# Mordentary/RayTracer-Cuda

Measured on AMD Instinct MI355X. Metric: Mrays/sec + frame wall-clock, Cornell+bunny 2560×1440 2000spp 20bounce, higher is better.
Workload: dtype f32

## Files before the change

### include/crt_hip.h

```cpp
#ifndef CRT_HIP_H
#define CRT_HIP_H

#include <stddef.h>
#include <stdint.h>

#ifdef __cplusplus
extern "C" {
#endif

#define CRT_ABI_VERSION 3

enum crt_status {
    CRT_OK = 0,
    CRT_ERR_INVALID_ARGUMENT = -1,
    CRT_ERR_HIP = -2,
    CRT_ERR_OUT_OF_MEMORY = -3,
    CRT_ERR_NO_DEVICE = -4,
    CRT_ERR_UNSUPPORTED = -5
};

enum crt_material_type { CRT_LAMBERTIAN = 0, CRT_METAL = 1, CRT_DIELECTRIC = 2, CRT_DIFFUSE_LIGHT = 3 };

typedef struct crt_material_desc {
    int32_t type;
// ... 250 lines not shown
int  crt_renderer_render(crt_renderer* r, const crt_scene* scene, int spp, int max_bounces, unsigned flags, void* stream);
int  crt_renderer_resolve(crt_renderer* r, float scale, void* stream);
int  crt_renderer_render_frame(crt_renderer* r, const crt_scene* scene, void* stream);
int  crt_renderer_synchronize(crt_renderer* r, void* stream);
int  crt_renderer_read_linear(crt_renderer* r, float* host_out);
int  crt_renderer_read_rgba8(crt_renderer* r, uint8_t* host_out);
int  crt_renderer_read_rng(crt_renderer* r, uint32_t* host_out);
int  crt_renderer_write_linear(crt_renderer* r, const float* host_in);
int  crt_renderer_get_counters(crt_renderer* r, crt_work_counters* out);
int  crt_renderer_get_schedule_stats(crt_renderer* r, unsigned long long* out3);
int  crt_renderer_get_section_profile(crt_renderer* r, unsigned long long* out7);
int  crt_renderer_get_section_profile_ex(crt_renderer* r, unsigned long long* out, int n);
float* crt_renderer_linear_device_ptr(crt_renderer* r);
int crt_renderer_attach_linear(crt_renderer* r, float* device_ptr);
uint8_t* crt_renderer_rgba_device_ptr(crt_renderer* r);
uint32_t* crt_renderer_rng_device_ptr(crt_renderer* r);
float crt_renderer_last_kernel_ms(crt_renderer* r);
int crt_renderer_last_schedule(crt_renderer* r, float out[4]);
int crt_renderer_last_timings(crt_renderer* r, float out[3]);
#define CRT_TIMING_RING 32
int crt_renderer_timing_history(crt_renderer* r, int back, float out[3]);
const char* crt_renderer_last_kernel_name(const crt_renderer* r);
int crt_renderer_last_launch_frozen(const crt_renderer* r);

int crt_build_mesh_bvh(int device, const float* positions, uint32_t vertex_count, uint32_t* indices,
                       int32_t* face_materials, uint32_t index_count, crt_bvh_node_desc* nodes, int32_t* node_count,
                       float mesh_box[6], float* build_ms);

int crt_selftest_math(const float* a, const float* b, int n, float* out, double* out_f64);
int crt_selftest_rcp(uint32_t lo_bits, uint32_t hi_bits, unsigned long long* mismatches, uint32_t* first_bad);
int crt_selftest_sqrt(uint32_t lo_bits, uint32_t hi_bits, unsigned long long* mismatches, uint32_t* first_bad);
int crt_selftest_unit(const float* in, int n, float* out);
int crt_selftest_uv_div(int dim, unsigned long long* mismatches);
int crt_selftest_scan(const int* in, int n_waves, int* out);
int crt_selftest_geometry(int kind, const float* in, int n, const crt_camera_desc* cam, int width, int height,
                          uint32_t* rng, float* out);
int crt_selftest_rng(unsigned long long seed, const unsigned long long* subseq, int n, int n_draw,
                     uint32_t* state_out , float* uniforms_out );
int crt_selftest_tile_schedule(crt_renderer* r, const uint32_t* pix_cost, int stride, int key_mode, int shard, int shards,
                               int xcd_regions, unsigned long long* stats_out);
int crt_selftest_pixel_order(crt_renderer* r, int kind, const uint32_t* in, int shard, int shards);
int crt_selftest_schedule_buffer(crt_renderer* r, int which, uint32_t* out, int64_t capacity, int64_t* n);

#ifdef __cplusplus
}
#endif
// ... 2 lines not shown
```

### raytracer-cuda_amd/crt_amd/__init__.py

```python
from __future__ import annotations

import ctypes as C
from dataclasses import dataclass

import numpy as np

from . import _lib
from ._lib import CameraDesc, CrtError, SceneDesc, SceneStats, WorkCounters, build, check, check_host

RENDER_ACCUMULATE = 1
RENDER_COUNT_WORK = 2

BENCH_CAMERA = dict(aspect=16.0 / 9.0, vfov=80.0, pos=(0.0, 0.0, 0.3), up=(0.0, 1.0, 0.0),
                    aperture=0.000001, focus=0.3, yaw=-90.0, pitch=0.0)


def _p(a: np.ndarray):
    return a.ctypes.data_as(C.c_void_p)


def camera(spp: int = 1, aspect=16.0 / 9.0, vfov=80.0, pos=(0.0, 0.0, 0.3), up=(0.0, 1.0, 0.0),
           aperture=0.000001, focus=0.3, yaw=-90.0, pitch=0.0) -> CameraDesc:
    d = CameraDesc()
    check_host(_lib.host().crth_camera(C.c_float(aspect), C.c_float(vfov), _p(np.asarray(pos, np.float32)),
# ... 334 lines not shown
    def _borrow(cls, handle, width: int, height: int, device: int, owner):
        r = cls.__new__(cls)
        r.h, r.width, r.height, r.device, r._owned, r._owner = C.c_void_p(handle), width, height, device, False, owner
        return r

    def close(self):
        if getattr(self, "h", None) and _lib is not None:
            if getattr(self, "_owned", True):
                _lib.hip().crt_renderer_destroy(self.h)
            self.h = None

    __del__ = close

    def init_rand(self, seed: int = 41, subsequence_base: int = 0, stream=None):
        check(_lib.hip().crt_renderer_init_rand(self.h, int(seed), int(subsequence_base), stream), "init_rand")

    def set_schedule(self, probe_spp: int = -1, min_spp: int = 64, tile_key: int = 2, probe_stride: int = 0):
        flags = ((int(tile_key) & 0xf) << 16) | ((int(probe_stride) & 0xf) << 20)
        check(_lib.hip().crt_renderer_set_schedule(self.h, int(probe_spp), int(min_spp), flags), "set_schedule")

    def set_critical_tiles(self, tiles: int = -1, lanes: int = 16):
        check(_lib.hip().crt_renderer_set_critical_tiles(self.h, int(tiles), int(lanes)), "set_critical_tiles")

    def set_top_levels(self, levels: int = -1):
        check(_lib.hip().crt_renderer_set_top_levels(self.h, int(levels)), "set_top_levels")

    def set_pixel_shard(self, shard: int = 0, shards: int = 1):
        check(_lib.hip().crt_renderer_set_pixel_shard(self.h, int(shard), int(shards)), "set_pixel_shard")

    def set_kernel_variant(self, variant: int):
        check(_lib.hip().crt_renderer_set_kernel_variant(self.h, int(variant)), "set_kernel_variant")

    def set_occupancy_target(self, waves_per_simd: int):
        check(_lib.hip().crt_renderer_set_occupancy_target(self.h, int(waves_per_simd)), "set_occupancy_target")

    def set_regen_threshold(self, lanes: int):
        check(_lib.hip().crt_renderer_set_regen_threshold(self.h, int(lanes)), "set_regen_threshold")

    def set_stack_lds(self, entries: int):
        check(_lib.hip().crt_renderer_set_stack_lds(self.h, int(entries)), "set_stack_lds")

    def set_camera(self, cam: CameraDesc):
        self._cam = cam
        check(_lib.hip().crt_renderer_set_camera(self.h, C.byref(cam)), "set_camera")

    def render(self, scene: Scene, spp: int, max_bounces: int = 20, accumulate=False, count_work=False, stream=None):
# ... 558 lines not shown
```

### raytracer-cuda_amd/crt_amd/_lib.py

```python
from __future__ import annotations

import ctypes as C
import os
import subprocess
from pathlib import Path

PKG_ROOT = Path(__file__).resolve().parents[1]
REPO = PKG_ROOT.parent
LIB_DIR = PKG_ROOT / "lib"
HIP_LIB = Path(os.environ["CRT_HIP_LIB"]) if os.environ.get("CRT_HIP_LIB") else LIB_DIR / "libcrt_hip.so"
HOST_LIB = Path(os.environ["CRT_HOST_LIB"]) if os.environ.get("CRT_HOST_LIB") else LIB_DIR / "libcrt_host.so"


class CrtError(RuntimeError):
    pass


def build(jobs: int = 8) -> None:
    subprocess.run(["make", "-C", str(PKG_ROOT), f"-j{jobs}", "all"], check=True)


class CameraDesc(C.Structure):
    _fields_ = [("origin", C.c_float * 3), ("lower_left", C.c_float * 3), ("horizontal", C.c_float * 3),
                ("vertical", C.c_float * 3), ("right", C.c_float * 3), ("up", C.c_float * 3),
# ... 135 lines not shown
    "crt_renderer_last_kernel_name", "crt_renderer_last_timings", "crt_renderer_last_schedule", "crt_renderer_timing_history",
    "crt_renderer_set_leaf_carry", "crt_renderer_set_xcd_regions", "crt_renderer_set_temporal_order",
    "crt_renderer_set_drain_threshold", "crt_renderer_set_wave_drain",
    "crt_renderer_attach_linear", "crt_renderer_set_kernel_variant", "crt_renderer_get_schedule_stats",
    "crt_renderer_set_regen_threshold", "crt_renderer_set_occupancy_target",
    "crt_build_mesh_bvh", "crt_renderer_set_schedule", "crt_renderer_set_critical_tiles", "crt_renderer_set_pixel_shard",
    "crt_renderer_set_top_levels",
    "crt_selftest_math", "crt_selftest_rng", "crt_selftest_geometry", "crt_selftest_scan", "crt_selftest_rcp",
    "crt_selftest_uv_div", "crt_selftest_sqrt", "crt_selftest_unit",
    "crt_trace_validate_rays", "crt_scene_export_identity", "crt_scene_trace", "crt_scene_occluded",
    "crt_scene_trace_device", "crt_scene_trace_last_stats",
    "crt_renderer_camera_rays_device", "crt_scene_path_step_device", "crt_scene_export_shade_rows",
    "crt_scene_path_advance_device", "crt_path_advance_entries", "crt_renderer_render_wavefront",
    "crt_scene_trace_indirect_device", "crt_scene_path_advance_indirect_device", "crt_renderer_render_wavefront_queued",
    "crt_scene_path_finish_device", "crt_renderer_render_wavefront_finish",
    "crt_selftest_tile_schedule", "crt_selftest_pixel_order", "crt_selftest_schedule_buffer",
    "crt_renderer_render_adaptive", "crt_renderer_resolve_adaptive", "crt_renderer_read_tile_spp",
    "crt_renderer_read_tile_error", "crt_renderer_read_adaptive_prev", "crt_selftest_adaptive_plan",
    "crt_renderer_compute_guides", "crt_renderer_denoise", "crt_renderer_resolve_denoised",
    "crt_renderer_read_denoised", "crt_renderer_read_guides", "crt_renderer_denoised_device_ptr", "crt_selftest_denoise",
    "crt_renderer_denoise_iteration_ms", "crt_debug_live_allocations", "crt_renderer_last_launch_frozen",
    "crt_renderer_reproject", "crt_renderer_reset_history", "crt_renderer_denoise_history", "crt_renderer_resolve_history",
    "crt_renderer_read_history", "crt_renderer_history_device_ptr", "crt_selftest_reproject",
]
OPTIONAL_SYMBOLS = ("crt_renderer_camera_rays_device", "crt_scene_path_step_device", "crt_scene_export_shade_rows",
                    "crt_scene_path_advance_device", "crt_path_advance_entries", "crt_renderer_render_wavefront",
                    "crt_scene_trace_indirect_device", "crt_scene_path_advance_indirect_device",
                    "crt_renderer_render_wavefront_queued",
                    "crt_scene_path_finish_device", "crt_renderer_render_wavefront_finish",
                    "crt_selftest_tile_schedule", "crt_selftest_pixel_order", "crt_selftest_schedule_buffer",
                    "crt_renderer_render_adaptive", "crt_renderer_resolve_adaptive", "crt_renderer_read_tile_spp",
                    "crt_renderer_read_tile_error", "crt_renderer_read_adaptive_prev", "crt_selftest_adaptive_plan",
                    "crt_renderer_compute_guides", "crt_renderer_denoise", "crt_renderer_resolve_denoised",
                    "crt_renderer_read_denoised", "crt_renderer_read_guides", "crt_renderer_denoised_device_ptr",
                    "crt_selftest_denoise", "crt_renderer_denoise_iteration_ms", "crt_debug_live_allocations",
                    "crt_renderer_last_launch_frozen",
                    "crt_renderer_reproject", "crt_renderer_reset_history", "crt_renderer_denoise_history",
                    "crt_renderer_resolve_history", "crt_renderer_read_history", "crt_renderer_history_device_ptr",
                    "crt_selftest_reproject")

HOST_SYMBOLS = [
    "crth_scene_load", "crth_scene_load_ex", "crth_scene_build_ms", "crth_scene_destroy", "crth_scene_desc", "crth_scene_upload", "crth_scene_upload_ex", "crth_scene_counts",
    "crth_scene_loader_arrays", "crth_camera", "crth_last_error", "crth_encode_image", "crth_write_image",
    "crth_build_mesh_bvh", "crth_camera_create", "crth_camera_update", "crth_camera_get", "crth_camera_destroy",
    "crth_viewer_create", "crth_viewer_frame", "crth_viewer_camera", "crth_viewer_renderer", "crth_viewer_destroy",
    "crth_viewer_set_reproject",
]

_hip = None
_host = None


def _bind_single_runtime() -> None:
    if os.environ.get("CRT_NO_TORCH") == "1":
        return
    try:
        import torch
    except Exception:
        pass


def hip():
# ... 64 lines not shown
            "crt_renderer_render_wavefront": ([P, P, i32, i32, C.c_uint, P, P, P], i32),
            "crt_scene_trace_indirect_device": ([P, P, P, C.c_int64, P, P, P, C.c_uint, P], i32),
            "crt_scene_path_advance_indirect_device": ([P, P, P, P, P, P, C.c_int64, i32, P, P, P, P, P, P, P, P], i32),
            "crt_renderer_render_wavefront_queued": ([P, P, i32, i32, C.c_uint, P, i32, P, P], i32),
            "crt_scene_path_finish_device": ([P, P, P, P, P, C.c_int64, i32, P, P, P, P, P], i32),
            "crt_renderer_render_wavefront_finish": ([P, P, i32, i32, C.c_uint, P, i32, C.c_int64, P, P], i32),
            "crt_selftest_tile_schedule": ([P, P, i32, i32, i32, i32, i32, P], i32),
            "crt_selftest_pixel_order": ([P, i32, P, i32, i32], i32),
            "crt_selftest_schedule_buffer": ([P, i32, P, C.c_int64, P], i32),
            "crt_renderer_render_adaptive": ([P, P, P, i32, C.c_uint, P, P], i32),
            "crt_renderer_resolve_adaptive": ([P, P], i32),
            "crt_renderer_read_tile_spp": ([P, P], i32), "crt_renderer_read_tile_error": ([P, P], i32),
            "crt_renderer_read_adaptive_prev": ([P, P], i32),
            "crt_selftest_adaptive_plan": ([P, P, P, P, i32, i32, f32, P, P], i32),
            "crt_renderer_compute_guides": ([P, P, P, P], i32),
            "crt_renderer_denoise": ([P, P, f32, P, P], i32),
            "crt_renderer_resolve_denoised": ([P, P], i32),
            "crt_renderer_read_denoised": ([P, P], i32), "crt_renderer_read_guides": ([P, P], i32),
            "crt_renderer_denoised_device_ptr": ([P], P),
            "crt_selftest_denoise": ([P, P, P, P, P], i32),
            "crt_renderer_denoise_iteration_ms": ([P, P], i32),
            "crt_debug_live_allocations": ([P, P], i32),
            "crt_renderer_last_launch_frozen": ([P], i32),
            "crt_renderer_reproject": ([P, P, f32, P, P], i32),
            "crt_renderer_reset_history": ([P], i32),
            "crt_renderer_denoise_history": ([P, P, P, P], i32),
            "crt_renderer_resolve_history": ([P, P], i32),
            "crt_renderer_read_history": ([P, P], i32),
            "crt_renderer_history_device_ptr": ([P], P),
            "crt_selftest_reproject": ([P, P, P, P, P, P, P, P], i32),
        }
        for name, (args, res) in sig.items():
            if os.environ.get("CRT_SKIP_ABI_CHECK") and not hasattr(L, name):
                continue
            if name in OPTIONAL_SYMBOLS and not hasattr(L, name):
                continue
            fn = getattr(L, name)
            fn.argtypes = args
            fn.restype = res
        if L.crt_abi_version() != ABI_VERSION and not os.environ.get("CRT_SKIP_ABI_CHECK"):
            raise CrtError(f"{HIP_LIB}: C ABI version {L.crt_abi_version()}, these bindings expect {ABI_VERSION} "
                           "(rebuild the library, or set CRT_SKIP_ABI_CHECK=1 for an A/B run of an older build)")
        _hip = L
    return _hip


# ... 56 lines not shown
```

### raytracer-cuda_amd/csrc/crt_hip.hip

```cpp
#include <hip/hip_runtime.h>

#include <algorithm>
#include <atomic>
#include <chrono>
#include <cstdio>
#include <cstdlib>
#include <cstring>
#include <memory>
#include <mutex>
#include <new>
#include <string>
#include <thread>
#include <type_traits>
#include <vector>

#include "crt_hip.h"
#include "crt_device.h"
#include "crt_devmem.h"
#include "crt_sah.h"
#include "crt/ParallelFor.h"

using namespace crt;

static thread_local std::string g_last_error;
// ... 28 lines not shown
    float sph2[2][12];
    unsigned* err;
    int width, height, spp, max_bounces;
    float rcp_w, rcp_h;
    int fast_uv;
    int accumulate;
    int regen_threshold;
    uint32_t* __restrict__ rng;
    float* __restrict__ sum;
    unsigned long long* __restrict__ counters;
    crt_camera_desc cam;
    const uint32_t* __restrict__ order;
    uint32_t* __restrict__ queue;
    int n_slots;
    int tiles_x;
    uint32_t* __restrict__ probe_cost;
    int probe_stride;
    uint32_t* __restrict__ pix_rays;
    int crit_tiles, crit_threshold;
    int drain_threshold;
    int wave_drain;
    int top_levels;
};

#ifdef CRT_PROFILE_LIVE
__device__ unsigned long long g_live_hist[16];
#endif
#ifdef CRT_PROFILE_PAIRS
__device__ unsigned long long g_pair_hist[32];
#endif

struct TraceCounts {
    uint32_t boxes, tris, spheres, step_slots, round_slots, trace_calls;
    uint64_t cyc_regen, cyc_step, cyc_round, passes;
    uint64_t cyc_shade, cyc_next;
    uint64_t cyc_sph;
    uint64_t cyc_setup, cyc_top, cyc_head;
#ifdef CRT_PROFILE_ROWS
    uint64_t cyc_rows, cyc_prims;
#endif
};
__device__ __forceinline__ uint64_t shader_clock() { return __builtin_amdgcn_s_memtime(); }
__device__ __forceinline__ uint64_t bcast64(uint64_t v, int lane) {
    return ((uint64_t)(uint32_t)__builtin_amdgcn_readlane((int)(v >> 32), lane) << 32) |
           (uint32_t)__builtin_amdgcn_readlane((int)(uint32_t)v, lane);
}
// ... 444 lines not shown
        const unsigned long long kk = L.key[lane];
        const float t = __uint_as_float((unsigned)(kk >> 32));
        const int rank = (int)(0xffffffffu - (unsigned)kk);
        if (kk != ~0ull && better(t, rank, closest, hit)) {
            closest = t;
            hit = rank;
        }
    }
}

#ifndef CRT_CHAIN_RHO
#define CRT_CHAIN_RHO 1.6
#endif
constexpr int STACK_LDS = 16;
#ifndef CRT_STACK6
#define CRT_STACK6 12
#endif
#ifndef CRT_STACK7
#define CRT_STACK7 8
#endif
constexpr int wide_stack_entries(int minw) { return minw >= 7 ? CRT_STACK7 : minw >= 6 ? CRT_STACK6 : STACK_LDS; }
constexpr int REGEN_THRESHOLD_WIDE = 44;
constexpr int WAVE_DRAIN = 48;

struct Wide4 {
    float tmin[4];
    bool hit[4];
};

constexpr float BOX_INV_CLAMP = 0x1p64f;
__device__ __forceinline__ V3 box_inv(V3 inv) {
    return v3(__builtin_amdgcn_fmed3f(inv.x, -BOX_INV_CLAMP, BOX_INV_CLAMP),
              __builtin_amdgcn_fmed3f(inv.y, -BOX_INV_CLAMP, BOX_INV_CLAMP),
              __builtin_amdgcn_fmed3f(inv.z, -BOX_INV_CLAMP, BOX_INV_CLAMP));
}
__device__ __forceinline__ V3 recip3_exact(V3 d) {
    const float ax = fabsf(d.x), ay = fabsf(d.y), az = fabsf(d.z);
    const bool ok = ax >= RCP_FAST_MIN && ax < RCP_FAST_MAX && ay >= RCP_FAST_MIN && ay < RCP_FAST_MAX &&
                    az >= RCP_FAST_MIN && az < RCP_FAST_MAX;
    if (__builtin_amdgcn_ballot_w64(!ok) == 0) return v3(rcp_newton(d.x), rcp_newton(d.y), rcp_newton(d.z));
    __asm__ volatile("");
    return v3(recip_exact_any(d.x), recip_exact_any(d.y), recip_exact_any(d.z));
}
__device__ __forceinline__ V3 sphere_inv(V3 d, V3 binv) {
    if (fabsf(binv.x) == BOX_INV_CLAMP || fabsf(binv.y) == BOX_INV_CLAMP || fabsf(binv.z) == BOX_INV_CLAMP)
        return v3(recip_exact_any(d.x), recip_exact_any(d.y), recip_exact_any(d.z));
// ... 725 lines not shown
    if (hit != h0 && hit >= 0) {
        if (P.n_ray_spheres == 2) {
            const int k = hit == __float_as_int(sph_lds[26]) ? 3 : 0;
            e0 = shd_lds[k];
            e1 = shd_lds[k + 1];
            inv_r = shd_lds[k + 2].x;
            staged = true;
        } else {
            const float4* Rh = P.shade + 3u * (uint32_t)hit;
            e0 = Rh[0];
            e1 = Rh[1];
        }
    }
    shade_rec(S, P, hit, closest, e0, e1, staged, inv_r);
}

#ifdef CRT_PROFILE_WAVE_TIMES
__device__ unsigned long long g_wave_prof[2 * 4 * 65536];
#endif
#ifdef CRT_PROFILE_CRIT_TRACE
__device__ unsigned long long g_crit_trace[2 * 16384];
__device__ unsigned g_wave_hw[2 * 4 * 65536];
#endif

template <int VARIANT> struct KernelShape { static constexpr int waves = VARIANT == 8 || VARIANT == 10 ? 1 : 4; };

template <bool COUNT, int VARIANT, int MINW>
__global__ __launch_bounds__(64 * KernelShape<VARIANT>::waves, MINW) void crt_render_kernel(RenderParams P) {
    constexpr bool FROZEN = VARIANT == 8 && !COUNT;
#include "crt_render_body.inc"
}
template <int VARIANT, int MINW>
__global__ __launch_bounds__(64 * KernelShape<VARIANT>::waves, MINW) void crt_render_open_kernel(RenderParams P) {
    static_assert(VARIANT == 8, "only the plain variant-8 kernels have twins");
    constexpr bool COUNT = false, FROZEN = false;
#include "crt_render_body.inc"
}

struct CompareParams {
    RenderParams A;
    const float4* __restrict__ nodes_b;
    const float4* __restrict__ prims_b;
    int n_nodes_b, n_layouts_b;
    int width_a, width_b;
    int sphere_first_b, n_spheres_b;
    const float4* chain_b;
// ... 1033 lines not shown
    PinnedBuf<unsigned long long> h_probe_stats;
    float last_schedule[4] = {0.f, 0.f, 0.f, 0.f};
    DevBuf<uint32_t> d_rng_cache;
    unsigned long long rng_cache_seed = 0, rng_cache_base = 0;
    bool rng_cache_valid = false;
    int probe_spp = -1;
    int probe_min_spp = 64;
    int tile_key_mode = 2;
    int n_cus = 0;
    int variant = -1;
    unsigned long long diag[3] = {0, 0, 0};
    unsigned long long prof[8] = {0, 0, 0, 0, 0, 0, 0, 0};
    int regen_threshold = 24;
    int regen_threshold_wide = REGEN_THRESHOLD_WIDE;
    int crit_tiles = -1;
    int tile_shard = 0, tile_shards = 1;
    int crit_threshold = 16;
    int top_levels = -1;
    int xcd_regions = 0;
    int probe_stride = 0;
    int temporal = 0;
    int drain_threshold = 0;
    int wave_drain = WAVE_DRAIN;
    DevBuf<uint32_t> d_pix_rays;
    DevBuf<uint32_t> d_tile_order;
    bool pix_rays_valid = false;
    int min_waves = 0;
    DevBuf<uint32_t> d_ovf;
    int stack_lds = STACK_LDS;
    float rcp_w = 1.f, rcp_h = 1.f;
    int fast_uv = 0;
    std::unique_ptr<WavefrontScratch> wavefront;
    std::unique_ptr<AdaptiveState> adaptive;
    std::unique_ptr<DenoiseState> denoise;
    std::unique_ptr<ReprojectState> reproject;
};

namespace {
int use_device(int dev) {
    int n = 0;
    HIP_TRY(hipGetDeviceCount(&n));
    if (n <= 0) return set_error(CRT_ERR_NO_DEVICE, "no HIP device visible");
    if (dev < 0 || dev >= n) return set_error(CRT_ERR_INVALID_ARGUMENT, "device ordinal out of range");
    HIP_TRY(hipSetDevice(dev));
    return CRT_OK;
}
// ... 542 lines not shown
static_assert(render_row_digits(8, true) == 55555677, "variant 8, counting");
static_assert(render_row_digits(10, false) == 55555677 && render_row_digits(10, true) == 55555677, "variant 10");
static_assert(render_row_digits(3, false) == 11145666 && render_row_digits(3, true) == 11145666, "variant 3");
static_assert(render_row_digits(2, false) == 11115668 && render_row_digits(2, true) == 11115668, "variant 2");
static_assert(render_row_digits(0, false) == 11111111 && render_row_digits(0, true) == 11111111, "variant 0");
static_assert(render_row_digits(1, false) == 11111111 && render_row_digits(1, true) == 11111111, "variant 1");

static bool render_launch_frozen(const RenderRow& row, bool cnt, const RenderParams& P, const crt_scene* S) {
    if (!row.open || cnt) return false;
    const int sd = wide_stack_entries(row.w);
    const bool own_bound = S->stack_cap == S->stack_bound;
    const bool stack = own_bound && (P.stack_lds == sd || (S->stack_cap < sd && P.stack_lds == S->stack_cap));
    return stack && P.top_levels == CRT_TOP_LEVELS && P.tree_spheres == 0 && P.n_ray_spheres == 2 && P.n_layouts == 1 &&
           !P.probe_cost && !P.pix_rays && P.wave_drain == WAVE_DRAIN && P.regen_threshold == REGEN_THRESHOLD_WIDE;
}

static int launch_render(crt_renderer* R, const RenderRow& row, bool cnt, dim3 grid, dim3 block, hipStream_t st,
                         const RenderParams& P, const crt_scene* S = nullptr) {
    std::snprintf(R->kernel_name, sizeof R->kernel_name, "crt_render_kernel<%s, %d, %d>", cnt ? "true" : "false",
                  row.variant, row.w);
    if (row.open && !S) return set_error(CRT_ERR_INVALID_ARGUMENT, "launch_render: a variant-8 launch needs its scene");
    R->last_frozen = render_launch_frozen(row, cnt, P, S) ? 1 : 0;
    HIP_TRY(hipEventRecord(R->ev_main, st));
    if (R->last_frozen) {
        RenderParams Q = P;
        Q.stack_lds = wide_stack_entries(row.w);
        hipLaunchKernelGGL(row.plain, grid, block, 0, st, Q);
    } else {
        hipLaunchKernelGGL(cnt ? row.counting : row.open ? row.open : row.plain, grid, block, 0, st, P);
    }
    return CRT_OK;
}

static int ensure_order_buffers(crt_renderer* R, hipStream_t st, size_t n_pix, int n_tiles, bool want_tile_key) {
    if (R->d_order && (R->d_tile_key || !want_tile_key)) return CRT_OK;
    HIP_TRY(hipStreamSynchronize(st));
    if (!R->d_order) {
        HIP_TRY(R->d_order.alloc(std::max(n_pix, (size_t)n_tiles * 64)));
        HIP_TRY(R->d_queue.alloc(1));
        HIP_TRY(R->d_tile_cost.alloc(n_pix));
        HIP_TRY(R->d_order_hist.alloc(ORDER_KEYS));
        HIP_TRY(hipDeviceGetAttribute(&R->n_cus, hipDeviceAttributeMultiprocessorCount, R->device));
    }
    if (want_tile_key && !R->d_tile_key) HIP_TRY(R->d_tile_key.alloc((size_t)n_tiles));
    return CRT_OK;
}

static int sort_descending(crt_renderer* R, hipStream_t st, const uint32_t* keys, int n, uint32_t* out) {
    const unsigned ob = (unsigned)((n + ORDER_ITEMS - 1) / ORDER_ITEMS);
    HIP_TRY(hipMemsetAsync(R->d_order_hist.get(), 0, ORDER_KEYS * 4, st));
    hipLaunchKernelGGL(crt_order_hist_kernel, dim3(ob), dim3(256), 0, st, keys, n, R->d_order_hist.get());
    hipLaunchKernelGGL(crt_order_scan_kernel, dim3(1), dim3(ORDER_KEYS), 0, st, R->d_order_hist.get());
    hipLaunchKernelGGL(crt_order_scatter_kernel, dim3(ob), dim3(256), 0, st, keys, n, R->d_order_hist.get(), out, 0u);
    return CRT_OK;
}

static int order_tiles_by_probe(crt_renderer* R, hipStream_t st, int stride, bool stats, int shard, int shards) {
    const size_t n_pix = (size_t)R->width * R->height;
    const int tiles_x = (R->width + 7) / 8, n_tiles = tiles_x * ((R->height + 7) / 8);
    const dim3 tgrid((n_tiles + 255) / 256), tblock(256);
    if (stats) {
        if (!R->d_probe_stats) {
            HIP_TRY(R->d_probe_stats.alloc(2));
            HIP_TRY(R->h_probe_stats.alloc(2));
// ... 113 lines not shown
        if (variant == 8) {
            P.crit_tiles = R->crit_tiles < 0 ? 4 * R->n_cus : R->crit_tiles;
            P.crit_threshold = R->crit_threshold;
        }
        if (auto_small) {
            HIP_TRY(hipStreamSynchronize(st));
            const double mx = (double)R->h_probe_stats.get()[0];
            const double mine = (double)R->h_probe_stats.get()[1] / shards;
            const double rho = mine > 0 ? mx * (4.0 * R->n_cus * 6) / mine : 0.0;
            if (rho > CRT_CHAIN_RHO) {
                occ = 4;
                P.stack_lds = stack_lds_for(R, S, occ);
            }
            R->last_schedule[0] = (float)rho;
            R->last_schedule[2] = (float)mx;
            R->last_schedule[3] = (float)(mine / std::max(1, n_tiles / shards));
        }
    } else if (shards > 1) {
        shard_tiles_in_row_order(R, st, n_tiles, shard, shards);
        P.order = R->d_order.get();
    }
    if (P.crit_tiles > 0) P.crit_tiles = (P.crit_tiles + shards - 1) / shards;
    if (variant == 8) R->last_schedule[1] = (float)occ;
    const dim3 tgrid((unsigned)((n_tiles - shard + shards - 1) / shards));
    return launch_render(R, RENDER_ROWS[render_row(variant, cnt, occ)], cnt, tgrid, dim3(64), st, P, S);
}

static int order_tile_slots(crt_renderer* R, hipStream_t st) {
    const size_t n_pix = (size_t)R->width * R->height;
    const int tiles_x = (R->width + 7) / 8, n_tiles = tiles_x * ((R->height + 7) / 8);
    const size_t n_tile_slots = (size_t)n_tiles * 64;
    if (R->temporal && !R->d_pix_rays) {
        HIP_TRY(hipStreamSynchronize(st));
        HIP_TRY(R->d_pix_rays.alloc(n_pix));
        HIP_TRY(R->d_tile_order.alloc((size_t)n_tiles));
        if (!R->d_tile_key) HIP_TRY(R->d_tile_key.alloc((size_t)n_tiles));
        R->pix_rays_valid = false;
    }
    const dim3 sgrid((unsigned)((n_tile_slots + 255) / 256));
    if (R->temporal && R->pix_rays_valid) {
        hipLaunchKernelGGL(crt_tile_cost_kernel, dim3((n_tiles + 255) / 256), dim3(256), 0, st, R->d_pix_rays.get(),
                           R->width, R->height, tiles_x, n_tiles, R->d_tile_order.get(), 0, 1, nullptr);
        hipLaunchKernelGGL(crt_tile_neighbour_kernel, dim3((n_tiles + 255) / 256), dim3(256), 0, st,
                           R->d_tile_order.get(), tiles_x, n_tiles, R->d_tile_key.get());
        if (int rc = sort_descending(R, st, R->d_tile_key.get(), n_tiles, R->d_tile_order.get())) return rc;
        hipLaunchKernelGGL(crt_expand_tile_order_kernel, sgrid, dim3(256), 0, st, R->d_tile_order.get(), R->d_order.get(),
// ... 208 lines not shown
int crt_renderer_get_section_profile(crt_renderer* R, unsigned long long* out7) {
    if (!R || !out7) return set_error(CRT_ERR_INVALID_ARGUMENT, "null argument");
    for (int i = 0; i < 7; ++i) out7[i] = R->prof[i];
    return CRT_OK;
}
int crt_renderer_get_section_profile_ex(crt_renderer* R, unsigned long long* out, int n) {
    if (!R || !out || n < 0) return set_error(CRT_ERR_INVALID_ARGUMENT, "bad argument");
    for (int i = 0; i < n && i < 8; ++i) out[i] = R->prof[i];
    return CRT_OK;
}
int crt_renderer_get_schedule_stats(crt_renderer* R, unsigned long long* out3) {
    if (!R || !out3) return set_error(CRT_ERR_INVALID_ARGUMENT, "null argument");
    out3[0] = R->diag[0]; out3[1] = R->diag[1]; out3[2] = R->diag[2];
    return CRT_OK;
}

float* crt_renderer_linear_device_ptr(crt_renderer* R) { return R ? R->d_sum : nullptr; }
uint8_t* crt_renderer_rgba_device_ptr(crt_renderer* R) { return R ? R->d_rgba.get() : nullptr; }
uint32_t* crt_renderer_rng_device_ptr(crt_renderer* R) { return R ? R->d_rng.get() : nullptr; }

const char* crt_renderer_last_kernel_name(const crt_renderer* R) { return R ? R->kernel_name : ""; }
int crt_renderer_last_launch_frozen(const crt_renderer* R) { return R ? R->last_frozen : 0; }

#ifdef CRT_PROFILE_PAIRS
extern "C" int crt_profile_pair_hist(unsigned long long* out32, int reset) {
    if (!out32) return set_error(CRT_ERR_INVALID_ARGUMENT, "bad argument");
    HIP_TRY(hipDeviceSynchronize());
    HIP_TRY(hipMemcpyFromSymbol(out32, HIP_SYMBOL(g_pair_hist), 32 * 8, 0, hipMemcpyDeviceToHost));
    if (reset) {
        static const unsigned long long zero[32] = {};
        HIP_TRY(hipMemcpyToSymbol(HIP_SYMBOL(g_pair_hist), zero, sizeof zero, 0, hipMemcpyHostToDevice));
    }
    return CRT_OK;
}
#endif
#ifdef CRT_PROFILE_LIVE
extern "C" int crt_profile_live_hist(unsigned long long* out16, int reset) {
    if (!out16) return set_error(CRT_ERR_INVALID_ARGUMENT, "bad argument");
    HIP_TRY(hipDeviceSynchronize());
    HIP_TRY(hipMemcpyFromSymbol(out16, HIP_SYMBOL(g_live_hist), 16 * 8, 0, hipMemcpyDeviceToHost));
    if (reset) {
        static const unsigned long long zero[16] = {};
        HIP_TRY(hipMemcpyToSymbol(HIP_SYMBOL(g_live_hist), zero, sizeof zero, 0, hipMemcpyHostToDevice));
    }
    return CRT_OK;
}
// ... 344 lines not shown
```

### raytracer-cuda_amd/csrc/crt_render_body.inc

```
    static_assert(!FROZEN || (VARIANT == 8 && !COUNT), "only the plain variant-8 kernels have a frozen twin");
    if constexpr (FROZEN) {
        constexpr int FROZEN_STACK = wide_stack_entries(MINW);
        __builtin_assume(P.stack_lds == FROZEN_STACK);
        __builtin_assume(P.top_levels == CRT_TOP_LEVELS);
        __builtin_assume(P.tree_spheres == 0);
        __builtin_assume(P.n_ray_spheres == 2);
        __builtin_assume(P.n_layouts == 1);
        __builtin_assume(P.probe_cost == nullptr);
        __builtin_assume(P.pix_rays == nullptr);
        __builtin_assume(P.wave_drain == WAVE_DRAIN);
        __builtin_assume(P.regen_threshold == REGEN_THRESHOLD_WIDE);
    }
#ifdef CRT_PROFILE_WAVE_TIMES
    const unsigned long long prof_t0 = __builtin_amdgcn_s_memrealtime();
#endif
#ifdef CRT_PROFILE_PASS
    const uint64_t prof_life0 = shader_clock();
#endif
    constexpr int WGW = KernelShape<VARIANT>::waves;
    constexpr bool PERSIST = VARIANT == 7;
    constexpr bool TILED = VARIANT == 8;
    constexpr bool TILES = TILED || VARIANT == 10;
    constexpr bool WIDE = VARIANT == 4 || PERSIST || TILED;
    using Lds = std::conditional_t<WIDE, WaveLdsWide, WaveLds>;
// ... 10 lines not shown
            const int k = threadIdx.x & 15;
            const int src = k < 4 ? k : k < 9 ? k + 1 : k == 9 ? 10 : k == 10 ? 4 : -1;
            sph_lds[threadIdx.x] = src < 0 ? 0.f : P.sph2[threadIdx.x >> 4][src];
        }
        if (threadIdx.x >= 32 && threadIdx.x < 38 && P.n_ray_spheres == 2) {
            const uint32_t q = threadIdx.x - 32, sp = q / 3;
            shd_lds[q] = P.shade[3u * (uint32_t)__float_as_int(P.sph2[sp][4]) + q % 3];
        }
        if (TOPN > 0 && threadIdx.x < 8u * TOPN) {
            const uint32_t m = threadIdx.x >> 3, k = threadIdx.x & 7;
            int n = 0;
            if (m > 0) {
                const float4 rm = node_row(P.nodes, node_base(0), 6);
                n = (int)(m - 1) < (__float_as_int(rm.y) & 0xff) ? __float_as_int(rm.x) + (int)(m - 1) : -1;
            }
            if (n >= 0 && n < P.n_nodes) top_lds[threadIdx.x] = node_row(P.nodes, node_base(n), k);
        }
        __syncthreads();
    }
    const int lane = threadIdx.x & 63;
    const int wave = __builtin_amdgcn_readfirstlane(threadIdx.x >> 6);
    int x, y;
    if (TILES) {
        const uint32_t t = P.order ? P.order[blockIdx.x] : blockIdx.x;
        x = (int)(t % (uint32_t)P.tiles_x) * 8 + (lane & 7);
        y = (int)(t / (uint32_t)P.tiles_x) * 8 + (lane >> 3);
    } else {
        x = blockIdx.x * 16 + (wave & 1) * 8 + (lane & 7);
        y = blockIdx.y * 16 + (wave >> 1) * 8 + (lane >> 3);
        if (VARIANT == 4 && P.probe_cost) {
            x *= P.probe_stride;
            y *= P.probe_stride;
        }
    }
    const bool valid = x < P.width && y < P.height;
    const int pix = valid ? y * P.width + x : 0;

    PathState S;
    S.s = Rng{0, 0, 0, 0, 0, 0};
    S.pixel = v3(0.f, 0.f, 0.f);
    S.o = v3(0, 0, 0); S.d = v3(0, 0, 1); S.thr = v3(1, 1, 1);
    S.remaining = 0; S.bounce = 0; S.need_new = true; S.rays = 0; S.paths = 0;
#ifdef CRT_PROFILE_LOOPS
    S.k1 = S.k2 = S.kr = 0;
    unsigned long long lp[8] = {0, 0, 0, 0, 0, 0, 0, 0};
#endif
#ifdef CRT_PROFILE_SITES
    S.site = 0;
    unsigned long long sites[12] = {0, 0, 0, 0, 0, 0, 0, 0, 0, 0, 0, 0};
#endif
    if (valid && !PERSIST) {
        const uint32_t* r = P.rng + 6 * (size_t)pix;
        S.s = rng_load(r);
        if (P.accumulate) S.pixel = v3(P.sum[3 * (size_t)pix], P.sum[3 * (size_t)pix + 1], P.sum[3 * (size_t)pix + 2]);
        S.remaining = P.spp;
    }
    const CamRegs C = cam_regs(P.cam, P.width, P.height, P.rcp_w, P.rcp_h, P.fast_uv);
    TraceCounts cnt{0, 0, 0, 0, 0, 0, 0, 0, 0, 0, 0, 0, 0, 0, 0, 0};
    uint32_t wave_rays = 0;

    if constexpr (VARIANT == 0) {
        for (;;) {
            if (!next_ray(S, C, x, y, P.max_bounces)) break;
            ++S.rays;
            float t;
            const int hit = trace<COUNT>(P.nodes, P.prims, P.n_nodes, layout_base(S.d, P.n_layouts, P.n_nodes), S.o,
                                         S.d, t, cnt);
            shade(S, P, hit, t);
        }
    } else if constexpr (PERSIST) {
        auto& L = lds[wave];
        uint32_t* stk = stack_lds + wave * SD * 64;
        const float INF = __builtin_inff();
        const size_t n_pix = (size_t)P.width * P.height;
        const uint32_t total_slots = (uint32_t)P.n_slots;
        const uint64_t below = (1ull << lane) - 1ull;
        bool live = false, has_result = false, have = false;
        int node = -1, sp = 0, hit = -1, px = 0, py = 0, ppix = 0;
// ... 79 lines not shown
                    if (COUNT) cnt.spheres += P.n_ray_spheres;
                    L.ray0[lane] = make_float4(S.o.x, S.o.y, S.o.z, S.d.x);
                    if (COUNT) cnt.trace_calls++;
                    if (TOPN > 0) top_steps<COUNT, TOPN>(P, top_lds, S.o, inv, rows, node, sp, cnt, stk, (size_t)ppix, n_pix);
                }
                if (!wave_ballot(live)) break;
            }
            if (COUNT) cnt.cyc_regen += shader_clock() - c0;
            traverse_step4<COUNT>(P, S.o, S.d, inv, rows, node, sp, closest, hit, cnt, L, stk, lane, (size_t)ppix, n_pix);
        }
    } else if constexpr (WIDE) {
        auto& L = lds[wave];
        uint32_t* stk = stack_lds + wave * SD * 64;
        const float INF = __builtin_inff();
        const size_t n_pix = (size_t)P.width * P.height;
        uint64_t live_mask = wave_ballot(true);
        bool has_result = false;
        int node = -1, sp = 0, hit = -1;
        float closest = INF;
        V3 inv = v3(0.f, 0.f, 0.f);
        uint32_t rows = 0;
        L.owner_at[lane] = 0;
        if (TILED && lane == 0) L.rays = 0;
        const int regen_t = (TILED && (int)blockIdx.x < P.crit_tiles) ? P.crit_threshold : P.regen_threshold;
        bool first_pass = true;
        constexpr bool PFV = TILED && MINW <= 4;
        float4 pf[PFV ? 7 : 1];
        int pf_node = -1;
#ifdef CRT_PROFILE_CRIT_TRACE
        uint32_t crit_iter = 0;
#endif
#ifdef CRT_PROFILE_LIVE
        uint64_t lh0 = 0, lh1 = 0, lh2 = 0, lh3 = 0, lh4 = 0, lh5 = 0, lh6 = 0, lh7 = 0, lh8 = 0;
        uint64_t lt_prev = shader_clock();
        int lb_prev = 8;
#endif
        constexpr bool TIME = COUNT || kProfilePass;
        for (;;) {
            const uint64_t h0 = kProfilePass ? shader_clock() : 0;
            const uint64_t parked_mask = live_mask & wave_ballot(node < 0);
            const int n_parked = __popcll(parked_mask);
            const int n_live = __popcll(live_mask);
#ifdef CRT_PROFILE_LIVE
            if (TILED) {
                const uint64_t lt = shader_clock(), dt = lt - lt_prev;
                lt_prev = lt;
                lh0 += lb_prev == 0 ? dt : 0; lh1 += lb_prev == 1 ? dt : 0; lh2 += lb_prev == 2 ? dt : 0;
// ... 160 lines not shown
            if (live) live = next_ray(S, C, x, y, P.max_bounces);
            if (!wave_ballot(live)) break;
            float t;
            const int hit = trace_coop<COUNT>(P.nodes, P.prims, P.n_nodes, layout_base(S.d, P.n_layouts, P.n_nodes),
                                              P.n_prims, P.err, S.o, S.d, live, t, cnt, lds[wave], lane);
            if (live) {
                ++S.rays;
                shade(S, P, hit, t);
            }
        }
    }

    if (((WIDE && !PERSIST) || VARIANT == 3) && P.probe_cost) {
        if (valid) P.probe_cost[pix] = COUNT ? (16u * S.rays + cnt.boxes + 4u * cnt.tris) >> 3 : S.rays;
        return;
    }
    if (valid && !PERSIST) {
        uint32_t* r = P.rng + 6 * (size_t)pix;
        rng_store(r, S.s);
        P.sum[3 * (size_t)pix] = S.pixel.x;
        P.sum[3 * (size_t)pix + 1] = S.pixel.y;
        P.sum[3 * (size_t)pix + 2] = S.pixel.z;
    }
    if constexpr (TILED) wave_rays = lds[0].rays;
    const uint64_t wr = TILED ? (uint64_t)wave_rays : wave_sum_u64(S.rays);
    if (COUNT) {
        const uint64_t wb = wave_sum_u64(cnt.boxes), wt = wave_sum_u64(cnt.tris);
        const uint64_t ws = wave_sum_u64(cnt.spheres), wp = wave_sum_u64(S.paths);
        if (lane == 0) {
            atomicAdd(&P.counters[1], (unsigned long long)wb);
            atomicAdd(&P.counters[2], (unsigned long long)wt);
            atomicAdd(&P.counters[3], (unsigned long long)ws);
            atomicAdd(&P.counters[4], (unsigned long long)wp);
            atomicAdd(&P.counters[5], 64ull * cnt.step_slots);
            atomicAdd(&P.counters[6], 64ull * cnt.round_slots + ((unsigned long long)cnt.trace_calls << 40));
            atomicAdd(&P.counters[8], (unsigned long long)cnt.cyc_regen);
            atomicAdd(&P.counters[9], (unsigned long long)cnt.cyc_step);
            atomicAdd(&P.counters[10], (unsigned long long)cnt.cyc_round);
            atomicAdd(&P.counters[11], (unsigned long long)cnt.passes);
            atomicAdd(&P.counters[12], 1ull);
            atomicAdd(&P.counters[13], (unsigned long long)cnt.cyc_shade);
            atomicAdd(&P.counters[14], (unsigned long long)cnt.cyc_next);
            atomicAdd(&P.counters[7], (unsigned long long)cnt.cyc_sph);
        }
    }
    if (lane == 0) atomicAdd(&P.counters[0], (unsigned long long)wr);
// ... 36 lines not shown
```

Measured before the change: 23180.

## Split expensive tiles' sample budget into tail-fill blocks to balance the tail

For variant-8 tiled launches, the first half of the cost-ordered tiles render only spp minus a delta of samples. Extra blocks appended to the grid render the remaining delta samples for those tiles once the head block has published a completion flag, and a second launch sweeps any tiles that were not filled in time. The aim is to break up the long-running expensive tiles so idle CUs at the end of the frame have work to do. In exchange it adds flag polling, an extra kernel launch, a memset and a small device-to-host copy per frame, and the head and tail passes must hand off RNG state and accumulated sums correctly.

```diff
diff --git a/include/crt_hip.h b/include/crt_hip.h
--- a/include/crt_hip.h
+++ b/include/crt_hip.h
@@ -296,6 +296,8 @@
 int crt_renderer_timing_history(crt_renderer* r, int back, float out[3]);
 const char* crt_renderer_last_kernel_name(const crt_renderer* r);
 int crt_renderer_last_launch_frozen(const crt_renderer* r);
+int crt_renderer_set_tail_fill(crt_renderer* r, int tiles, int spp);
+int crt_renderer_last_tail_fill(crt_renderer* r, int out[4]);
 
 int crt_build_mesh_bvh(int device, const float* positions, uint32_t vertex_count, uint32_t* indices,
                        int32_t* face_materials, uint32_t index_count, crt_bvh_node_desc* nodes, int32_t* node_count,
diff --git a/raytracer-cuda_amd/crt_amd/__init__.py b/raytracer-cuda_amd/crt_amd/__init__.py
--- a/raytracer-cuda_amd/crt_amd/__init__.py
+++ b/raytracer-cuda_amd/crt_amd/__init__.py
@@ -380,6 +380,14 @@
     def set_critical_tiles(self, tiles: int = -1, lanes: int = 16):
         check(_lib.hip().crt_renderer_set_critical_tiles(self.h, int(tiles), int(lanes)), "set_critical_tiles")
 
+    def set_tail_fill(self, tiles: int = -1, spp: int = 0):
+        check(_lib.require("crt_renderer_set_tail_fill")(self.h, int(tiles), int(spp)), "set_tail_fill")
+
+    def last_tail_fill(self) -> dict:
+        a = (C.c_int * 4)()
+        check(_lib.require("crt_renderer_last_tail_fill")(self.h, a), "last_tail_fill")
+        return dict(zip(("tiles", "spp", "in_launch", "swept"), (int(v) for v in a)))
+
     def set_top_levels(self, levels: int = -1):
         check(_lib.hip().crt_renderer_set_top_levels(self.h, int(levels)), "set_top_levels")
 
diff --git a/raytracer-cuda_amd/crt_amd/_lib.py b/raytracer-cuda_amd/crt_amd/_lib.py
--- a/raytracer-cuda_amd/crt_amd/_lib.py
+++ b/raytracer-cuda_amd/crt_amd/_lib.py
@@ -181,6 +181,7 @@
     "crt_renderer_denoise_iteration_ms", "crt_debug_live_allocations", "crt_renderer_last_launch_frozen",
     "crt_renderer_reproject", "crt_renderer_reset_history", "crt_renderer_denoise_history", "crt_renderer_resolve_history",
     "crt_renderer_read_history", "crt_renderer_history_device_ptr", "crt_selftest_reproject",
+    "crt_renderer_set_tail_fill", "crt_renderer_last_tail_fill",
 ]
 OPTIONAL_SYMBOLS = ("crt_renderer_camera_rays_device", "crt_scene_path_step_device", "crt_scene_export_shade_rows",
                     "crt_scene_path_advance_device", "crt_path_advance_entries", "crt_renderer_render_wavefront",
@@ -196,7 +197,8 @@
                     "crt_renderer_last_launch_frozen",
                     "crt_renderer_reproject", "crt_renderer_reset_history", "crt_renderer_denoise_history",
                     "crt_renderer_resolve_history", "crt_renderer_read_history", "crt_renderer_history_device_ptr",
-                    "crt_selftest_reproject")
+                    "crt_selftest_reproject",
+                    "crt_renderer_set_tail_fill", "crt_renderer_last_tail_fill")
 
 HOST_SYMBOLS = [
     "crth_scene_load", "crth_scene_load_ex", "crth_scene_build_ms", "crth_scene_destroy", "crth_scene_desc", "crth_scene_upload", "crth_scene_upload_ex", "crth_scene_counts",
@@ -307,6 +309,8 @@
             "crt_renderer_denoise_iteration_ms": ([P, P], i32),
             "crt_debug_live_allocations": ([P, P], i32),
             "crt_renderer_last_launch_frozen": ([P], i32),
+            "crt_renderer_set_tail_fill": ([P, i32, i32], i32),
+            "crt_renderer_last_tail_fill": ([P, P], i32),
             "crt_renderer_reproject": ([P, P, f32, P, P], i32),
             "crt_renderer_reset_history": ([P], i32),
             "crt_renderer_denoise_history": ([P, P, P, P], i32),
diff --git a/raytracer-cuda_amd/csrc/crt_hip.hip b/raytracer-cuda_amd/csrc/crt_hip.hip
--- a/raytracer-cuda_amd/csrc/crt_hip.hip
+++ b/raytracer-cuda_amd/csrc/crt_hip.hip
@@ -74,6 +74,11 @@
     int wave_drain;
     int top_levels;
 };
+__device__ __forceinline__ uint32_t* fill_flags(const RenderParams& P) { return P.queue + 2; }
+__device__ __forceinline__ uint32_t* fill_done(const RenderParams& P) { return P.queue + (P.n_slots ? 0 : 1); }
+__device__ __forceinline__ uint32_t fill_heads(const RenderParams& P) { return (uint32_t)P.n_slots; }
+__device__ __forceinline__ uint32_t fill_tiles(const RenderParams& P) { return (uint32_t)P.drain_threshold; }
+__device__ __forceinline__ int fill_spp(const RenderParams& P) { return P.probe_stride; }
 
 #ifdef CRT_PROFILE_LIVE
 __device__ unsigned long long g_live_hist[16];
@@ -564,6 +569,10 @@
 constexpr int wide_stack_entries(int minw) { return minw >= 7 ? CRT_STACK7 : minw >= 6 ? CRT_STACK6 : STACK_LDS; }
 constexpr int REGEN_THRESHOLD_WIDE = 44;
 constexpr int WAVE_DRAIN = 48;
+#ifndef CRT_FILL_AUTO
+#define CRT_FILL_AUTO 1
+#endif
+constexpr int CRT_FILL_TILES_NUM = 1, CRT_FILL_TILES_DEN = 2, CRT_FILL_SPP_DEN = 16, CRT_FILL_MIN_SPP = 12;
 
 struct Wide4 {
     float tmin[4];
@@ -1335,6 +1344,47 @@
 __device__ unsigned long long g_crit_trace[2 * 16384];
 __device__ unsigned g_wave_hw[2 * 4 * 65536];
 #endif
+
+struct FillNote {
+    uint32_t* flag;
+    uint32_t* done;
+    uint32_t set;
+};
+__device__ __forceinline__ bool fill_prologue(const RenderParams& P, uint32_t b, uint32_t& rank, int& spp, int& accumulate,
+                                              FillNote* note) {
+    rank = b;
+    spp = P.spp;
+    accumulate = P.accumulate;
+    uint32_t set = 0;
+    if (P.queue) {
+        if (b >= fill_heads(P)) {
+            rank = b - fill_heads(P);
+            const uint32_t f = __hip_atomic_load(fill_flags(P) + rank, __ATOMIC_ACQUIRE, __HIP_MEMORY_SCOPE_AGENT);
+            if (__builtin_amdgcn_readfirstlane(f) != 1u) return false;
+            spp = fill_spp(P);
+            accumulate = 1;
+            set = 2;
+        } else if (b < fill_tiles(P)) {
+            spp = P.spp - fill_spp(P);
+            set = 1;
+        }
+    }
+    if (threadIdx.x == 0) {
+        note->flag = set ? fill_flags(P) + rank : nullptr;
+        note->done = set ? fill_done(P) : nullptr;
+        note->set = set;
+    }
+    return true;
+}
+__device__ __forceinline__ void fill_epilogue(const FillNote* note, int lane) {
+    const uint32_t set = __builtin_amdgcn_readfirstlane(note->set);
+    if (set == 0) return;
+    __syncthreads();
+    if (lane == 0) {
+        __hip_atomic_store(note->flag, set, __ATOMIC_RELEASE, __HIP_MEMORY_SCOPE_AGENT);
+        if (set == 2u) atomicAdd(note->done, 1u);
+    }
+}
 
 template <int VARIANT> struct KernelShape { static constexpr int waves = VARIANT == 8 || VARIANT == 10 ? 1 : 4; };
 
@@ -2414,6 +2464,11 @@
     int temporal = 0;
     int drain_threshold = 0;
     int wave_drain = WAVE_DRAIN;
+    int fill_tiles = -1, fill_spp = 0;
+    DevBuf<uint32_t> d_fill;
+    PinnedBuf<uint32_t> h_fill;
+    int last_fill[2] = {0, 0};
+    hipEvent_t last_fill_ev = nullptr;
     DevBuf<uint32_t> d_pix_rays;
     DevBuf<uint32_t> d_tile_order;
     bool pix_rays_valid = false;
@@ -3002,13 +3057,24 @@
     if (row.open && !S) return set_error(CRT_ERR_INVALID_ARGUMENT, "launch_render: a variant-8 launch needs its scene");
     R->last_frozen = render_launch_frozen(row, cnt, P, S) ? 1 : 0;
     HIP_TRY(hipEventRecord(R->ev_main, st));
-    if (R->last_frozen) {
-        RenderParams Q = P;
-        Q.stack_lds = wide_stack_entries(row.w);
-        hipLaunchKernelGGL(row.plain, grid, block, 0, st, Q);
-    } else {
-        hipLaunchKernelGGL(cnt ? row.counting : row.open ? row.open : row.plain, grid, block, 0, st, P);
-    }
+    RenderParams Q = P;
+    if (R->last_frozen) Q.stack_lds = wide_stack_entries(row.w);
+    const RenderKernel kernel = R->last_frozen ? row.plain : cnt ? row.counting : row.open ? row.open : row.plain;
+    R->last_fill[0] = R->last_fill[1] = 0;
+    if (row.variant != 8 || !P.queue) {
+        hipLaunchKernelGGL(kernel, grid, block, 0, st, Q);
+        return CRT_OK;
+    }
+    const int k = P.drain_threshold, delta = P.probe_stride;
+    HIP_TRY(hipMemsetAsync(R->d_fill.get(), 0, ((size_t)k + 2) * sizeof(uint32_t), st));
+    Q.n_slots = (int)grid.x;
+    hipLaunchKernelGGL(kernel, dim3(grid.x + (unsigned)k), block, 0, st, Q);
+    Q.n_slots = 0;
+    hipLaunchKernelGGL(kernel, dim3((unsigned)k), block, 0, st, Q);
+    HIP_TRY(hipMemcpyAsync(R->h_fill.get(), R->d_fill.get(), 2 * sizeof(uint32_t), hipMemcpyDeviceToHost, st));
+    R->last_fill[0] = k;
+    R->last_fill[1] = delta;
+    R->last_fill_ev = R->ev1;
     return CRT_OK;
 }
 
@@ -3020,6 +3086,8 @@
         HIP_TRY(R->d_queue.alloc(1));
         HIP_TRY(R->d_tile_cost.alloc(n_pix));
         HIP_TRY(R->d_order_hist.alloc(ORDER_KEYS));
+        HIP_TRY(R->d_fill.alloc((size_t)n_tiles + 2));
+        HIP_TRY(R->h_fill.alloc(2));
         HIP_TRY(hipDeviceGetAttribute(&R->n_cus, hipDeviceAttributeMultiprocessorCount, R->device));
     }
     if (want_tile_key && !R->d_tile_key) HIP_TRY(R->d_tile_key.alloc((size_t)n_tiles));
@@ -3179,6 +3247,21 @@
     }
     if (P.crit_tiles > 0) P.crit_tiles = (P.crit_tiles + shards - 1) / shards;
     if (variant == 8) R->last_schedule[1] = (float)occ;
+    if (variant == 8 && !cnt && shards == 1 && R->fill_tiles != 0) {
+        int k = R->fill_tiles, delta = R->fill_spp;
+        if (k < 0) {
+            const bool on = CRT_FILL_AUTO && P.order && probe_spp_for(R, spp) > 0 && !R->min_waves && occ == 7;
+            k = on ? (int)((long long)n_tiles * CRT_FILL_TILES_NUM / CRT_FILL_TILES_DEN) : 0;
+            delta = spp / CRT_FILL_SPP_DEN;
+            if (delta < CRT_FILL_MIN_SPP) k = 0;
+        }
+        k = std::min(k, n_tiles);
+        if (k > 0 && delta >= 1 && delta <= spp - 1) {
+            P.queue = R->d_fill.get();
+            P.drain_threshold = k;
+            P.probe_stride = delta;
+        }
+    }
     const dim3 tgrid((unsigned)((n_tiles - shard + shards - 1) / shards));
     return launch_render(R, RENDER_ROWS[render_row(variant, cnt, occ)], cnt, tgrid, dim3(64), st, P, S);
 }
@@ -3433,6 +3516,24 @@
 const char* crt_renderer_last_kernel_name(const crt_renderer* R) { return R ? R->kernel_name : ""; }
 int crt_renderer_last_launch_frozen(const crt_renderer* R) { return R ? R->last_frozen : 0; }
 
+int crt_renderer_set_tail_fill(crt_renderer* R, int tiles, int spp) {
+    if (!R) return set_error(CRT_ERR_INVALID_ARGUMENT, "null renderer");
+    R->fill_tiles = tiles < 0 ? -1 : tiles;
+    R->fill_spp = tiles > 0 ? spp : 0;
+    return CRT_OK;
+}
+
+int crt_renderer_last_tail_fill(crt_renderer* R, int out[4]) {
+    if (!R || !out) return set_error(CRT_ERR_INVALID_ARGUMENT, "null argument");
+    out[0] = R->last_fill[0]; out[1] = R->last_fill[1]; out[2] = out[3] = 0;
+    if (out[0] == 0) return CRT_OK;
+    HIP_TRY(hipSetDevice(R->device));
+    HIP_TRY(hipEventSynchronize(R->last_fill_ev));
+    out[2] = (int)R->h_fill.get()[0];
+    out[3] = (int)R->h_fill.get()[1];
+    return CRT_OK;
+}
+
 #ifdef CRT_PROFILE_PAIRS
 extern "C" int crt_profile_pair_hist(unsigned long long* out32, int reset) {
     if (!out32) return set_error(CRT_ERR_INVALID_ARGUMENT, "bad argument");
diff --git a/raytracer-cuda_amd/csrc/crt_render_body.inc b/raytracer-cuda_amd/csrc/crt_render_body.inc
--- a/raytracer-cuda_amd/csrc/crt_render_body.inc
+++ b/raytracer-cuda_amd/csrc/crt_render_body.inc
@@ -1,4 +1,10 @@
     static_assert(!FROZEN || (VARIANT == 8 && !COUNT), "only the plain variant-8 kernels have a frozen twin");
+    uint32_t rank = 0;
+    int blk_spp = 0, blk_accumulate = 0;
+    __shared__ FillNote fill_note;
+    if constexpr (VARIANT == 8) {
+        if (!fill_prologue(P, blockIdx.x, rank, blk_spp, blk_accumulate, &fill_note)) return;
+    }
     if constexpr (FROZEN) {
         constexpr int FROZEN_STACK = wide_stack_entries(MINW);
         __builtin_assume(P.stack_lds == FROZEN_STACK);
@@ -56,7 +62,8 @@
     const int wave = __builtin_amdgcn_readfirstlane(threadIdx.x >> 6);
     int x, y;
     if (TILES) {
-        const uint32_t t = P.order ? P.order[blockIdx.x] : blockIdx.x;
+        const uint32_t b = TILED ? rank : blockIdx.x;
+        const uint32_t t = P.order ? P.order[b] : b;
         x = (int)(t % (uint32_t)P.tiles_x) * 8 + (lane & 7);
         y = (int)(t / (uint32_t)P.tiles_x) * 8 + (lane >> 3);
     } else {
@@ -86,8 +93,9 @@
     if (valid && !PERSIST) {
         const uint32_t* r = P.rng + 6 * (size_t)pix;
         S.s = rng_load(r);
-        if (P.accumulate) S.pixel = v3(P.sum[3 * (size_t)pix], P.sum[3 * (size_t)pix + 1], P.sum[3 * (size_t)pix + 2]);
-        S.remaining = P.spp;
+        if (TILED ? blk_accumulate : P.accumulate)
+            S.pixel = v3(P.sum[3 * (size_t)pix], P.sum[3 * (size_t)pix + 1], P.sum[3 * (size_t)pix + 2]);
+        S.remaining = TILED ? blk_spp : P.spp;
     }
     const CamRegs C = cam_regs(P.cam, P.width, P.height, P.rcp_w, P.rcp_h, P.fast_uv);
     TraceCounts cnt{0, 0, 0, 0, 0, 0, 0, 0, 0, 0, 0, 0, 0, 0, 0, 0};
@@ -213,7 +221,7 @@
         uint32_t rows = 0;
         L.owner_at[lane] = 0;
         if (TILED && lane == 0) L.rays = 0;
-        const int regen_t = (TILED && (int)blockIdx.x < P.crit_tiles) ? P.crit_threshold : P.regen_threshold;
+        const int regen_t = (TILED && (int)rank < P.crit_tiles) ? P.crit_threshold : P.regen_threshold;
         bool first_pass = true;
         constexpr bool PFV = TILED && MINW <= 4;
         float4 pf[PFV ? 7 : 1];
@@ -420,6 +428,7 @@
         P.sum[3 * (size_t)pix + 1] = S.pixel.y;
         P.sum[3 * (size_t)pix + 2] = S.pixel.z;
     }
+    if constexpr (TILED) fill_epilogue(&fill_note, lane);
     if constexpr (TILED) wave_rays = lds[0].rays;
     const uint64_t wr = TILED ? (uint64_t)wave_rays : wave_sum_u64(S.rays);
     if (COUNT) {
```

Result: faster. 23770, median of 6 (+2.5%).
